# HKUST-Aerial-Robotics/Omni-swarm

Measured on NVIDIA H100. Metric: keyframes/sec (SuperPoint+NetVLAD+match), higher is better.
Workload: dtype f32

## Files before the change

omni-swarm_b200/csrc/conv_umma.cu:

```cuda
#include <cuda.h>
#include <cuda_fp16.h>
#include <cmath>
#include "common.cuh"
#include "kernels.cuh"
#include "conv_umma.cuh"
#include "umma_ptx.cuh"

namespace osb {

constexpr int UM_TH = 8, UM_TW = 16;
constexpr int UM_KC = 64;
constexpr int UM_ROW = UM_TW * 128;

constexpr int UM_A_SLOT = (UM_TH + 2) * UM_ROW;
constexpr int UM_A_SLOTS = 2;
constexpr int UM_CONSUMERS = 256;
constexpr int UM_THREADS = UM_CONSUMERS + 128;
constexpr int UM_PRODUCER_REGS = 40, UM_CONSUMER_REGS = 232;
static_assert(128 * UM_PRODUCER_REGS + UM_CONSUMERS * UM_CONSUMER_REGS <= 65536, "register file");
template <int N, bool FP16 = false>
struct UmmaCfg {
  static constexpr int PLANES = FP16 ? 1 : 2;
  static constexpr int A_SLOTS = FP16 ? 4 : UM_A_SLOTS;
  static constexpr int A_RING = A_SLOTS * PLANES * UM_A_SLOT;
  static constexpr int B_BYTES = N * 128;
  static constexpr int B_SLOT = PLANES * B_BYTES;
  static constexpr int B_SLOTS = FP16 ? ((N <= 64) ? 12 : (N <= 80) ? 10 : 8) : ((N <= 64) ? 6 : (N <= 80) ? 5 : 4);
  static constexpr int SMEM_BYTES = A_RING + B_SLOTS * B_SLOT + 1024  + 256 ;
  static_assert(SMEM_BYTES <= 227 * 1024, "shared-memory plan exceeds the 227 KB of an H100 block");
  static_assert(2 * (A_SLOTS + B_SLOTS) * 8 <= 256, "barriers exceed their 256 bytes");
};
template <bool FP16 = false>
struct R64Cfg {
  static constexpr int PLANES = FP16 ? 1 : 2;
  static constexpr int A_SLOTS = FP16 ? 6 : UM_A_SLOTS;
  static constexpr int A_RING = A_SLOTS * PLANES * UM_A_SLOT;
  static constexpr int W_PLANE = 64 * 128;
  static constexpr int W_SLOT = PLANES * W_PLANE;
  static constexpr int SMEM_BYTES = A_RING + 9 * W_SLOT + 1024  + 256 ;
  static_assert(SMEM_BYTES <= 227 * 1024, "shared-memory plan exceeds the 227 KB of an H100 block");
  static_assert((3 * A_SLOTS + 9) * 8 <= 256, "barriers exceed their 256 bytes");
};

struct UmmaArgs {
  const float* bias;
  __half* out_hi;
  __half* out_lo;
  float* out_f32;
  int H, W, B;
  int ks;
  int cin_slabs;
  int out_c;
  int out_cstride;
  float inv_scale;
  float out_scale;
  int relu;
  int n_off;
  int pool;
  int n_split;
  int epi;
};

__device__ __forceinline__ void quad_transpose(uint32_t (&v)[4], int t4) {
  uint32_t o[4];
#pragma unroll
  for (int k = 0; k < 4; ++k) o[k] = (k == t4) ? v[k] : 0u;
#pragma unroll
  for (int r = 1; r < 4; ++r) {
    const int send = (t4 - r) & 3, from = (t4 + r) & 3;
    uint32_t s = v[0];
#pragma unroll
    for (int k = 1; k < 4; ++k) s = (send == k) ? v[k] : s;
    const uint32_t got = __shfl_sync(0xffffffffu, s, (threadIdx.x & 28) | from);
#pragma unroll
    for (int k = 0; k < 4; ++k) o[k] = (from == k) ? got : o[k];
  }
#pragma unroll
  for (int k = 0; k < 4; ++k) v[k] = o[k];
}

template <int N, bool SPLIT, bool FP16 = false>
__global__ void __launch_bounds__(UM_THREADS, 1)
conv_umma_kernel(const __grid_constant__ CUtensorMap tm_a_hi, const __grid_constant__ CUtensorMap tm_a_lo,
                 const __grid_constant__ CUtensorMap tm_w_hi, const __grid_constant__ CUtensorMap tm_w_lo, UmmaArgs P) {
  using Cfg = UmmaCfg<N, FP16>;
  constexpr int AS = Cfg::A_SLOTS, BS = Cfg::B_SLOTS, A_STRIDE = Cfg::PLANES * UM_A_SLOT;
  extern __shared__ uint8_t smem_raw[];
  const uint32_t smem_base = (smem_u32(smem_raw) + 1023u) & ~1023u;
  const uint32_t b_base = smem_base + Cfg::A_RING;
  const uint32_t bar_base = b_base + BS * Cfg::B_SLOT;
  auto a_full = [&](int s) { return bar_base + 8u * s; };
  auto a_empty = [&](int s) { return bar_base + 8u * (AS + s); };
  auto b_full = [&](int s) { return bar_base + 8u * (2 * AS + s); };
  auto b_empty = [&](int s) { return bar_base + 8u * (2 * AS + BS + s); };

  const int lane = threadIdx.x & 31;
  const int tiles_x = (P.W + UM_TW - 1) / UM_TW, tiles_y = (P.H + UM_TH - 1) / UM_TH;
  const int n_tiles = P.B * tiles_x * tiles_y;
  const int n_split = SPLIT ? P.n_split : 1;
  const int n_items = n_tiles * n_split;
  const int halo = P.ks / 2;
  const uint32_t a_box_bytes = (uint32_t)(UM_TH + 2 * halo) * UM_ROW;

  if (threadIdx.x == 0) {
    for (int s = 0; s < AS; ++s) { mbar_init(a_full(s), 1); mbar_init(a_empty(s), 2); }
    for (int s = 0; s < BS; ++s) { mbar_init(b_full(s), 1); mbar_init(b_empty(s), 2); }
    asm volatile("fence.mbarrier_init.release.cluster;" ::: "memory");
  }
  __syncthreads();
  asm volatile("griddepcontrol.launch_dependents;" ::: "memory");

  if (threadIdx.x >= UM_CONSUMERS) {
    const int pt = threadIdx.x - UM_CONSUMERS;
    setmaxnreg_dec<UM_PRODUCER_REGS>();
    asm volatile("griddepcontrol.wait;" ::: "memory");
    if (pt < 32 && elect_one()) {
      int as = 0; uint32_t aph = 0;
      int bs = 0; uint32_t bph = 0;
      for (int item = blockIdx.x; item < n_items; item += gridDim.x) {
        const int tile = SPLIT ? item / n_split : item, n_off = SPLIT ? P.n_off + (item % n_split) * N : P.n_off;
        const int tx = tile % tiles_x, ty = (tile / tiles_x) % tiles_y, b = tile / (tiles_x * tiles_y);
        const int x0 = tx * UM_TW, y0 = ty * UM_TH;
        for (int kx = 0; kx < P.ks; ++kx) {
          for (int cs = 0; cs < P.cin_slabs; ++cs) {
            mbar_wait(a_empty(as), aph ^ 1);
            const uint32_t sa = smem_base + as * A_STRIDE;
            mbar_expect_tx(a_full(as), Cfg::PLANES * a_box_bytes);
            tma_load_4d(sa, &tm_a_hi, a_full(as), cs * UM_KC, x0 + kx - halo, y0 - halo, b);
            if constexpr (!FP16) tma_load_4d(sa + UM_A_SLOT, &tm_a_lo, a_full(as), cs * UM_KC, x0 + kx - halo, y0 - halo, b);
            if (++as == AS) { as = 0; aph ^= 1; }
            for (int ky = 0; ky < P.ks; ++ky) {
              mbar_wait(b_empty(bs), bph ^ 1);
              const uint32_t sb = b_base + bs * Cfg::B_SLOT;
              mbar_expect_tx(b_full(bs), Cfg::B_SLOT);
              tma_load_3d(sb, &tm_w_hi, b_full(bs), cs * UM_KC, n_off, ky * P.ks + kx);
              if constexpr (!FP16) tma_load_3d(sb + Cfg::B_BYTES, &tm_w_lo, b_full(bs), cs * UM_KC, n_off, ky * P.ks + kx);
              if (++bs == BS) { bs = 0; bph ^= 1; }
            }
          }
        }
      }
    }
  } else {
    setmaxnreg_inc<UM_CONSUMER_REGS>();
    const int cw = threadIdx.x >> 7;
    const int wq = (threadIdx.x >> 5) & 3;
    const int col = lane >> 2, t4 = lane & 3;
    const bool signaller = (threadIdx.x & 127) == 0;
    int as = 0; uint32_t aph = 0;
    int bs = 0; uint32_t bph = 0;
    auto release = [&](int a_slot, int b_slot) {
      if (!signaller) return;
      if (a_slot >= 0) mbar_arrive(a_empty(a_slot));
      if (b_slot >= 0) mbar_arrive(b_empty(b_slot));
    };
    for (int item = blockIdx.x; item < n_items; item += gridDim.x) {
      const int tile = SPLIT ? item / n_split : item, n_off = SPLIT ? P.n_off + (item % n_split) * N : P.n_off;
      float acc[N / 2], cross[FP16 ? 1 : N / 2];
#pragma unroll
      for (int i = 0; i < N / 2; ++i) { acc[i] = 0.f; if constexpr (!FP16) cross[i] = 0.f; }
      uint32_t scale_d = 0;
      int pend_a = -1, pend_b = -1;
      for (int kx = 0; kx < P.ks; ++kx) {
        for (int cs = 0; cs < P.cin_slabs; ++cs) {
          mbar_wait(a_full(as), aph);
          const uint32_t sa = smem_base + as * A_STRIDE + cw * 1024;
          for (int ky = 0; ky < P.ks; ++ky) {
            mbar_wait(b_full(bs), bph);
            const uint32_t sb = b_base + bs * Cfg::B_SLOT;
            const int b_slot = bs;
            if (++bs == BS) { bs = 0; bph ^= 1; }
            const uint64_t a_hi = wgmma_desc_sw128(sa + ky * UM_ROW, UM_ROW);
            const uint64_t a_lo = wgmma_desc_sw128(sa + UM_A_SLOT + ky * UM_ROW, UM_ROW);
            const uint64_t b_hi = wgmma_desc_sw128(sb, 1024), b_lo = wgmma_desc_sw128(sb + Cfg::B_BYTES, 1024);
#pragma unroll
            for (int i = 0; i < N / 2; ++i) { fence_operand(acc[i]); if constexpr (!FP16) fence_operand(cross[i]); }
            wgmma_fence();
#pragma unroll
            for (int k = 0; k < UM_KC / 16; ++k) {
              const uint64_t adv = (uint64_t)(k * 32 >> 4);
// ... 126 lines not shown
          float f[4];
#pragma unroll
          for (int i = 0; i < 4; ++i) {
            float a = value(4 * j + i, c + (i & 1));
            if (P.relu) a = fmaxf(a, 0.f);
            if (P.relu == 2) a = fminf(a, 6.f);
            f[i] = a;
          }
          if (P.pool) {
            float m0 = fmaxf(f[0], f[2]), m1 = fmaxf(f[1], f[3]);
            m0 = fmaxf(m0, __shfl_xor_sync(0xffffffffu, m0, 4));
            m1 = fmaxf(m1, __shfl_xor_sync(0xffffffffu, m1, 4));
            if (pool_writer) store(ppix, c, m0, m1);
          } else {
            if (in0) store(pix0, c, f[0], f[1]);
            if (in1) store(pix1, c, f[2], f[3]);
          }
        }
      }
    }
  }
}

template <bool FP16 = false>
__global__ void __launch_bounds__(UM_THREADS, 1)
conv_res64_kernel(const __grid_constant__ CUtensorMap tm_a_hi, const __grid_constant__ CUtensorMap tm_a_lo,
                  const __grid_constant__ CUtensorMap tm_w_hi, const __grid_constant__ CUtensorMap tm_w_lo, UmmaArgs P) {
  using Cfg = R64Cfg<FP16>;
  constexpr int AS = Cfg::A_SLOTS, A_STRIDE = Cfg::PLANES * UM_A_SLOT;
  constexpr int R64_W_PLANE = Cfg::W_PLANE, R64_W_SLOT = Cfg::W_SLOT;
  extern __shared__ uint8_t smem_raw[];
  const uint32_t smem_base = (smem_u32(smem_raw) + 1023u) & ~1023u;
  const uint32_t w_base = smem_base + Cfg::A_RING;
  const uint32_t bar_base = w_base + 9 * R64_W_SLOT;
  auto a_full = [&](int g, int s) { return bar_base + 8u * (g * AS + s); };
  auto a_empty = [&](int s) { return bar_base + 8u * (2 * AS + s); };
  auto w_full = [&](int t) { return bar_base + 8u * (3 * AS + t); };

  const int lane = threadIdx.x & 31;
  const int tiles_x = (P.W + UM_TW - 1) / UM_TW, tiles_y = (P.H + UM_TH - 1) / UM_TH;
  const int n_tiles = P.B * tiles_x * tiles_y;

  if (threadIdx.x == 0) {
    for (int s = 0; s < AS; ++s) { mbar_init(a_full(0, s), 1); mbar_init(a_full(1, s), 1); mbar_init(a_empty(s), 1); }
    for (int t = 0; t < 9; ++t) mbar_init(w_full(t), 1);
    asm volatile("fence.mbarrier_init.release.cluster;" ::: "memory");
// ... 60 lines not shown
#pragma unroll
          for (int k = 0; k < UM_KC / 16; ++k) {
            const uint64_t adv = (uint64_t)(k * 32 >> 4);
            Wgmma<128>::mma(acc, w_hi + adv, x_hi + adv, scale_d);
            if constexpr (!FP16) {
              Wgmma<128>::mma(cross, w_lo + adv, x_hi + adv, scale_d);
              Wgmma<128>::mma(cross, w_hi + adv, x_lo + adv, 1u);
            }
            scale_d = 1;
          }
          wgmma_commit();
#pragma unroll
          for (int k = 0; k < 64; ++k) { fence_operand(acc[k]); if constexpr (!FP16) fence_operand(cross[k]); }
          wgmma_wait<1>();
          if (signaller && pend >= 0) mbar_arrive(a_empty(pend));
          pend = (ky == 2) ? as : -1;
        }
      }
      wgmma_wait<0>();
      if (signaller) mbar_arrive(a_empty(pend));
#pragma unroll
      for (int k = 0; k < 64; ++k) { fence_operand(acc[k]); if constexpr (!FP16) fence_operand(cross[k]); }

      const int tx = tile % tiles_x, ty = (tile / tiles_x) % tiles_y, b = tile / (tiles_x * tiles_y);
      const int x0 = tx * UM_TW, y0 = ty * UM_TH;
      auto value = [&](int k, int h) {
        float a;
        if constexpr (FP16) a = fmaf(acc[k], P.inv_scale, bias[h]);
        else a = fmaf(acc[k] + cross[k], P.inv_scale, bias[h]);
        if (P.relu) a = fmaxf(a, 0.f);
        if (P.relu == 2) a = fminf(a, 6.f);
        return a;
      };
      auto split_t = [&](float v0, float v1, uint32_t& th, uint32_t& tl) {
        const float s0 = v0 * P.out_scale, s1 = v1 * P.out_scale;
        const __half2 hp = __floats2half2_rn(s0, s1);
        if constexpr (FP16) {
          th = movmatrix_trans(*reinterpret_cast<const uint32_t*>(&hp));
        } else {
          const float2 hf = __half22float2(hp);
          const __half2 lp = __floats2half2_rn(s0 - hf.x, s1 - hf.y);
          th = movmatrix_trans(*reinterpret_cast<const uint32_t*>(&hp));
          tl = movmatrix_trans(*reinterpret_cast<const uint32_t*>(&lp));
        }
      };
#pragma unroll
      for (int h = 0; h < 2; ++h) {
        const int cb = 16 * w + 8 * h;
        if (cb >= P.out_c) continue;
        const int c_own = P.n_off + cb + r, c_st = P.n_off + cb + 2 * t4;
        if (P.pool) {
          const int Hp = P.H >> 1, Wp = P.W >> 1;
#pragma unroll
          for (int py = 0; py < UM_TH / 2; ++py) {
            float m[2];
#pragma unroll
            for (int k = 0; k < 2; ++k) {
              const int j = 4 * py + k;
              m[k] = fmaxf(fmaxf(value(4 * j + 2 * h, h), value(4 * (j + 2) + 2 * h, h)),
                           fmaxf(value(4 * j + 2 * h + 1, h), value(4 * (j + 2) + 2 * h + 1, h)));
            }
            const int gpy = ty * (UM_TH / 2) + py;
            if (P.out_f32) {
#pragma unroll
              for (int k = 0; k < 2; ++k) {
                const int gpx = tx * (UM_TW / 2) + 4 * k + t4;
                if (gpy < Hp && gpx < Wp)
                  P.out_f32[(((size_t)b * Hp + gpy) * Wp + gpx) * P.out_cstride + c_own] = m[k];
              }
            } else {
              uint32_t th, tl;
              split_t(m[0], m[1], th, tl);
              const int gpx = tx * (UM_TW / 2) + 4 * (r & 1) + (r >> 1);
              if (gpy < Hp && gpx < Wp) {
                const size_t o = (((size_t)b * Hp + gpy) * Wp + gpx) * P.out_cstride + c_st;
                *reinterpret_cast<uint32_t*>(P.out_hi + o) = th;
                if constexpr (!FP16) *reinterpret_cast<uint32_t*>(P.out_lo + o) = tl;
              }
            }
          }
        } else {
#pragma unroll
          for (int j = 0; j < 16; ++j) {
            const int gy = y0 + (j >> 1), xb = x0 + 8 * (j & 1);
            const float v0 = value(4 * j + 2 * h, h), v1 = value(4 * j + 2 * h + 1, h);
            if (P.out_f32) {
              const int gx = xb + 2 * t4;
              const size_t o = (((size_t)b * P.H + gy) * P.W + gx) * P.out_cstride + c_own;
              if (gy < P.H && gx < P.W) P.out_f32[o] = v0;
              if (gy < P.H && gx + 1 < P.W) P.out_f32[o + P.out_cstride] = v1;
            } else {
              uint32_t th, tl;
              split_t(v0, v1, th, tl);
              const int gx = xb + r;
              if (gy < P.H && gx < P.W) {
                const size_t o = (((size_t)b * P.H + gy) * P.W + gx) * P.out_cstride + c_st;
                *reinterpret_cast<uint32_t*>(P.out_hi + o) = th;
                if constexpr (!FP16) *reinterpret_cast<uint32_t*>(P.out_lo + o) = tl;
              }
            }
          }
        }
      }
    }
  }
}

template <bool FP16>
__device__ __forceinline__ void split_store8(__half* hi, __half* lo, const float* f, float scale) {
  uint32_t h[4], l[4];
#pragma unroll
  for (int i = 0; i < 4; ++i) {
    const float s0 = f[2 * i] * scale, s1 = f[2 * i + 1] * scale;
    const __half h0 = __float2half_rn(s0), h1 = __float2half_rn(s1);
    h[i] = (uint32_t)__half_as_ushort(h0) | ((uint32_t)__half_as_ushort(h1) << 16);
    if constexpr (!FP16) {
      const __half l0 = __float2half_rn(s0 - __half2float(h0)), l1 = __float2half_rn(s1 - __half2float(h1));
      l[i] = (uint32_t)__half_as_ushort(l0) | ((uint32_t)__half_as_ushort(l1) << 16);
    }
  }
  *reinterpret_cast<uint4*>(hi) = make_uint4(h[0], h[1], h[2], h[3]);
  if constexpr (!FP16) *reinterpret_cast<uint4*>(lo) = make_uint4(l[0], l[1], l[2], l[3]);
}

constexpr int CF_TW = 32, CF_TH = 8;
template <bool FP16 = false>
// ... 110 lines not shown
    bp[o] = bias[o];
    for (int c = 0; c < cin; ++c)
      for (int t = 0; t < L->taps; ++t) {
        const float s = w_oihw[((size_t)o * cin + c) * L->taps + t] * w_scale;
        const __half h = __float2half_rn(s);
        if (!std::isfinite(__half2float(h))) {
          char buf[192];
          snprintf(buf, sizeof(buf), "weight %g (output %d, input %d, tap %d) is outside the split-fp16 range: "
                   "|w| * %g must be below 65520", (double)w_oihw[((size_t)o * cin + c) * L->taps + t], o, c, t,
                   (double)w_scale);
          set_error("umma_layer_upload", buf);
          return OSB_ERR_INVALID;
        }
        const size_t idx = ((size_t)t * L->n_pad + o) * cin + c;
        hi[idx] = h;
        lo[idx] = __float2half_rn(s - __half2float(h));
      }
  }
  OSB_TRY(res.upload(&L->w_hi, hi.data(), n));
  OSB_TRY(res.upload(&L->w_lo, lo.data(), n));
  OSB_TRY(res.upload(&L->bias, bp.data(), L->n_pad));
  const uint64_t dims[3] = {(uint64_t)cin, (uint64_t)L->n_pad, (uint64_t)L->taps};
  const uint64_t strides[2] = {(uint64_t)cin * 2, (uint64_t)cin * L->n_pad * 2};
  const uint32_t box[3] = {UM_KC, (uint32_t)std::min(L->n_pad, 256), 1};
  OSB_TRY(umma_make_tmap(&L->tm_hi, L->w_hi, 3, dims, strides, box));
  OSB_TRY(umma_make_tmap(&L->tm_lo, L->w_lo, 3, dims, strides, box));
  if (L->n_pad >= 256) {
    const uint32_t box128[3] = {UM_KC, 128, 1};
    OSB_TRY(umma_make_tmap(&L->tm_hi128, L->w_hi, 3, dims, strides, box128));
    OSB_TRY(umma_make_tmap(&L->tm_lo128, L->w_lo, 3, dims, strides, box128));
  }
  return OSB_OK;
}

osb_status umma_act_maps(CUtensorMap* hi, CUtensorMap* lo, __half* p_hi, __half* p_lo, int B, int H, int W, int C,
                         int ks) {
  const uint64_t dims[4] = {(uint64_t)C, (uint64_t)W, (uint64_t)H, (uint64_t)B};
  const uint64_t strides[3] = {(uint64_t)C * 2, (uint64_t)W * C * 2, (uint64_t)H * W * C * 2};
  const uint32_t box[4] = {UM_KC, UM_TW, (uint32_t)(UM_TH + 2 * (ks / 2)), 1};
  osb_status s;
  if ((s = umma_make_tmap(hi, p_hi, 4, dims, strides, box)) != OSB_OK) return s;
  return umma_make_tmap(lo, p_lo, 4, dims, strides, box);
}

static const bool g_conv_pdl = [] { const char* e = getenv("OSB_CONV_PDL"); return e && atoi(e) != 0; }();

template <auto kernel>
static osb_status launch_persistent(int smem_bytes, const CUtensorMap& a_hi, const CUtensorMap& a_lo,
                                    const CUtensorMap& w_hi, const CUtensorMap& w_lo, const UmmaArgs& P, cudaStream_t st,
                                    int max_ctas) {
  OSB_SMEM_OPT_IN(kernel, smem_bytes);
  const int tiles = P.B * cdiv(P.W, UM_TW) * cdiv(P.H, UM_TH) * P.n_split;
  const int grid = std::min(tiles, persistent_ctas(max_ctas));
  cudaLaunchConfig_t cfg = {};
  cudaLaunchAttribute attr[1];
  cfg.gridDim = dim3(grid); cfg.blockDim = dim3(UM_THREADS); cfg.dynamicSmemBytes = smem_bytes; cfg.stream = st;
  attr[0].id = cudaLaunchAttributeProgrammaticStreamSerialization;
  attr[0].val.programmaticStreamSerializationAllowed = g_conv_pdl ? 1 : 0;
  cfg.attrs = attr; cfg.numAttrs = 1;
  OSB_CUDA(cudaLaunchKernelEx(&cfg, kernel, a_hi, a_lo, w_hi, w_lo, P));
  g_launches.fetch_add(1, std::memory_order_relaxed);
  return OSB_OK;
}

template <int N, bool SPLIT = false, bool FP16 = false>
static osb_status launch_umma(const CUtensorMap& a_hi, const CUtensorMap& a_lo, const UmmaLayer& L, const UmmaArgs& P,
                              cudaStream_t st, int max_ctas, bool box128 = false) {
  return launch_persistent<conv_umma_kernel<N, SPLIT, FP16>>(UmmaCfg<N, FP16>::SMEM_BYTES, a_hi, a_lo,
                           box128 ? L.tm_hi128 : L.tm_hi, box128 ? L.tm_lo128 : L.tm_lo, P, st, max_ctas);
}

static bool precision_fp16(int precision) { return precision == OSB_PRECISION_FP16; }

static UmmaArgs umma_args(const UmmaLayer& L, int B, int H, int W, float act_scale) {
  UmmaArgs P = {};
  P.bias = L.bias; P.H = H; P.W = W; P.B = B; P.ks = L.ks; P.cin_slabs = L.cin / UM_KC;
  P.inv_scale = 1.0f / (act_scale * L.w_scale); P.n_split = 1;
  return P;
}

template <bool FP16>
static osb_status umma_conv_launch(const UmmaLayer& L, const CUtensorMap& a_hi, const CUtensorMap& a_lo, UmmaArgs& P,
                                   cudaStream_t st, int max_ctas) {
  switch (L.n_pad) {
    case 64:
      if (L.ks == 3 && L.cin == UM_KC)
        return launch_persistent<conv_res64_kernel<FP16>>(R64Cfg<FP16>::SMEM_BYTES, a_hi, a_lo, L.tm_hi, L.tm_lo, P, st,
                                                          max_ctas);
      return launch_umma<64, false, FP16>(a_hi, a_lo, L, P, st, max_ctas);
    case 80: return launch_umma<80, false, FP16>(a_hi, a_lo, L, P, st, max_ctas);
    case 128: return launch_umma<128, false, FP16>(a_hi, a_lo, L, P, st, max_ctas);
    case 256:
    case 512:
      P.n_split = L.n_pad / 128;
      return launch_umma<128, true, FP16>(a_hi, a_lo, L, P, st, max_ctas, true);
  }
  set_error("umma_conv_forward", "unsupported N");
  return OSB_ERR_INVALID;
}

osb_status umma_conv_forward(const UmmaLayer& L, const CUtensorMap& a_hi, const CUtensorMap& a_lo, int B, int H, int W,
                             float act_scale, __half* out_hi, __half* out_lo, float* out_f32, int out_c, int out_cstride,
                             float out_scale, int relu, int pool, cudaStream_t st, int max_ctas, int precision) {
  OSB_REQUIRE(!pool || (H % 2 == 0 && W % 2 == 0), "fused max-pool needs even H and W");
  OSB_REQUIRE(out_c % 16 == 0 && out_c <= L.n_pad && out_cstride % 8 == 0, "tensor-core conv: bad output channel layout");
  UmmaArgs P = umma_args(L, B, H, W, act_scale);
  P.out_hi = out_hi; P.out_lo = out_lo; P.out_f32 = out_f32; P.out_c = out_c; P.out_cstride = out_cstride;
  P.out_scale = out_scale; P.relu = relu; P.pool = pool;
  return precision_fp16(precision) ? umma_conv_launch<true>(L, a_hi, a_lo, P, st, max_ctas)
                                   : umma_conv_launch<false>(L, a_hi, a_lo, P, st, max_ctas);
}

osb_status umma_conv_softmax_forward(const UmmaLayer& L, const CUtensorMap& a_hi, const CUtensorMap& a_lo, int B, int H, int W,
                                     float act_scale, float* semi, cudaStream_t st, int max_ctas, int precision) {
  OSB_REQUIRE(L.n_pad == 80 && L.cout == 65 && L.ks == 1, "fused detector head expects the 65-logit 1x1 layer");
  UmmaArgs P = umma_args(L, B, H, W, act_scale);
  P.out_f32 = semi; P.out_c = 80; P.out_cstride = 80; P.out_scale = 1.f; P.epi = 1;
  return precision_fp16(precision) ? launch_umma<80, false, true>(a_hi, a_lo, L, P, st, max_ctas)
                                   : launch_umma<80>(a_hi, a_lo, L, P, st, max_ctas);
}

template <bool FP16 = false>
__global__ void dwconv3x3_split_kernel(const float* __restrict__ w, const float* __restrict__ bias,
                                       const float* __restrict__ x, __half* __restrict__ out_hi,
                                       __half* __restrict__ out_lo, int H, int W, int Ho, int Wo, int C, int stride,
                                       float out_scale, int64_t total) {
  const int64_t i = (int64_t)blockIdx.x * blockDim.x + threadIdx.x;
  if (i >= total) return;
  const int C8 = C >> 3;
  const int c = (int)(i % C8) * 8;
  int64_t p = i / C8;
  const int ox = (int)(p % Wo); p /= Wo;
  const int oy = (int)(p % Ho);
  const int b = (int)(p / Ho);
  float a[8];
#pragma unroll
  for (int j = 0; j < 8; ++j) a[j] = 0.f;
#pragma unroll
  for (int ky = 0; ky < 3; ++ky)
#pragma unroll
    for (int kx = 0; kx < 3; ++kx) {
// ... 230 lines not shown
```

omni-swarm_b200/csrc/conv_umma.cuh:

```cuda
#pragma once
#include <cuda.h>
#include <cuda_fp16.h>
#include "common.cuh"

namespace osb {

struct UmmaLayer {
  int cin = 0, cout = 0, n_pad = 0, ks = 1, taps = 1;
  float w_scale = 1.f;
  __half *w_hi = nullptr, *w_lo = nullptr;
  float* bias = nullptr;
  CUtensorMap tm_hi, tm_lo;
  CUtensorMap tm_hi128, tm_lo128;
};

osb_status umma_layer_upload(Resources& res, UmmaLayer* L, const float* w_oihw, const float* bias, int cin, int cout,
                             int ks, float w_scale);
osb_status umma_act_maps(CUtensorMap* hi, CUtensorMap* lo, __half* p_hi, __half* p_lo, int B, int H, int W, int C,
                         int ks);
osb_status umma_conv_forward(const UmmaLayer& L, const CUtensorMap& a_hi, const CUtensorMap& a_lo, int B, int H, int W,
                             float act_scale, __half* out_hi, __half* out_lo, float* out_f32, int out_c, int out_cstride,
                             float out_scale, int relu, int pool, cudaStream_t st, int max_ctas = 0,
                             int precision = OSB_PRECISION_SPLIT_FP16);
osb_status umma_conv_softmax_forward(const UmmaLayer& L, const CUtensorMap& a_hi, const CUtensorMap& a_lo, int B, int H, int W,
                                     float act_scale, float* semi, cudaStream_t st, int max_ctas = 0,
                                     int precision = OSB_PRECISION_SPLIT_FP16);
osb_status umma_first_forward(const float* w_tap_cout, const float* bias, const float* lut, const uint8_t* img,
                              __half* out_hi, __half* out_lo, int B, int H, int W, float out_scale, cudaStream_t st,
                              int precision = OSB_PRECISION_SPLIT_FP16);
osb_status umma_make_tmap(CUtensorMap* tm, void* base, int rank, const uint64_t* dims, const uint64_t* strides_bytes,
                          const uint32_t* box);
osb_status umma_dwconv_forward(const float* w_tap_c, const float* bias, const float* x, __half* out_hi, __half* out_lo,
                               int B, int H, int W, int C, int stride, float out_scale, cudaStream_t st, bool s1x4 = true,
                               int precision = OSB_PRECISION_SPLIT_FP16);
}
```

omni-swarm_b200/csrc/umma_ptx.cuh:

```cuda
#pragma once
#include <cuda.h>
#include <cuda_fp16.h>
#include <stdint.h>

namespace osb {

__device__ __forceinline__ uint32_t smem_u32(const void* p) { return (uint32_t)__cvta_generic_to_shared(p); }
__device__ __forceinline__ void mbar_init(uint32_t bar, uint32_t count) {
  asm volatile("mbarrier.init.shared::cta.b64 [%0], %1;" ::"r"(bar), "r"(count) : "memory");
}
__device__ __forceinline__ void mbar_expect_tx(uint32_t bar, uint32_t bytes) {
  asm volatile("mbarrier.arrive.expect_tx.shared::cta.b64 _, [%0], %1;" ::"r"(bar), "r"(bytes) : "memory");
}
__device__ __forceinline__ void mbar_arrive(uint32_t bar) {
  asm volatile("mbarrier.arrive.shared::cta.b64 _, [%0];" ::"r"(bar) : "memory");
}
__device__ __forceinline__ void mbar_wait(uint32_t bar, uint32_t parity) {
  uint32_t done;
  uint32_t spins = 0;
  do {
    asm volatile("{\n\t.reg .pred p;\n\tmbarrier.try_wait.parity.shared::cta.b64 p, [%1], %2;\n\tselp.u32 %0, 1, 0, p;\n\t}"
                 : "=r"(done) : "r"(bar), "r"(parity) : "memory");
#ifdef OSB_MBAR_DEBUG
    if (!done && ++spins > (1u << 22)) {
      if (blockIdx.x == 0 && (threadIdx.x & 31) == 0)
        printf("mbar_wait stalled: block %d thread %d barrier +%u parity %u\n", blockIdx.x, threadIdx.x, bar & 0xFFFFu, parity);
      return;
    }
#else
    if (!done && ++spins > (1u << 24)) __trap();
#endif
  } while (!done);
}
__device__ __forceinline__ void tma_load_4d(uint32_t dst, const CUtensorMap* tm, uint32_t bar, int c0, int c1, int c2, int c3) {
  asm volatile("cp.async.bulk.tensor.4d.shared::cluster.global.tile.mbarrier::complete_tx::bytes [%0], [%1, {%3, %4, %5, %6}], [%2];"
               ::"r"(dst), "l"(tm), "r"(bar), "r"(c0), "r"(c1), "r"(c2), "r"(c3) : "memory");
}
__device__ __forceinline__ void tma_load_3d(uint32_t dst, const CUtensorMap* tm, uint32_t bar, int c0, int c1, int c2) {
  asm volatile("cp.async.bulk.tensor.3d.shared::cluster.global.tile.mbarrier::complete_tx::bytes [%0], [%1, {%3, %4, %5}], [%2];"
               ::"r"(dst), "l"(tm), "r"(bar), "r"(c0), "r"(c1), "r"(c2) : "memory");
}
__device__ __forceinline__ bool elect_one() {
  uint32_t pred = 0;
  asm volatile("{\n\t.reg .pred p;\n\telect.sync _|p, 0xffffffff;\n\tselp.u32 %0, 1, 0, p;\n\t}" : "=r"(pred));
  return pred != 0;
}

__device__ __forceinline__ uint64_t wgmma_desc_sw128(uint32_t saddr, uint32_t sbo_bytes) {
  return (uint64_t)((saddr >> 4) & 0x3FFF) | (1ull << 16) | ((uint64_t)((sbo_bytes >> 4) & 0x3FFF) << 32) | (1ull << 62);
}
template <int R> __device__ __forceinline__ void setmaxnreg_dec() { asm volatile("setmaxnreg.dec.sync.aligned.u32 %0;" ::"n"(R)); }
template <int R> __device__ __forceinline__ void setmaxnreg_inc() { asm volatile("setmaxnreg.inc.sync.aligned.u32 %0;" ::"n"(R)); }
__device__ __forceinline__ void wgmma_fence() { asm volatile("wgmma.fence.sync.aligned;" ::: "memory"); }
__device__ __forceinline__ void wgmma_commit() { asm volatile("wgmma.commit_group.sync.aligned;" ::: "memory"); }
template <int N> __device__ __forceinline__ void wgmma_wait() { asm volatile("wgmma.wait_group.sync.aligned %0;" ::"n"(N) : "memory"); }
__device__ __forceinline__ void fence_operand(float& r) { asm volatile("" : "+f"(r)::"memory"); }
__device__ __forceinline__ uint32_t movmatrix_trans(uint32_t a) {
  uint32_t d;
  asm volatile("movmatrix.sync.aligned.m8n8.trans.b16 %0, %1;" : "=r"(d) : "r"(a));
  return d;
}

template <int W> struct Wgmma;
template <> struct Wgmma<64> {
  static __device__ __forceinline__ void mma(float* d, uint64_t a, uint64_t b, uint32_t scale_d) {
    asm volatile("{\n\t.reg .pred p;\n\tsetp.ne.b32 p, %34, 0;\n\t"
                 "wgmma.mma_async.sync.aligned.m64n64k16.f32.f16.f16 {%0, %1, %2, %3, %4, %5, %6, %7, %8, %9, %10, %11, %12, %13, %14, %15, %16, %17, %18, %19, %20, %21, %22, %23, %24, %25, %26, %27, %28, %29, %30, %31}, %32, %33, p, 1, 1, 0, 0;\n\t}"
                 : "+f"(d[0]), "+f"(d[1]), "+f"(d[2]), "+f"(d[3]), "+f"(d[4]), "+f"(d[5]), "+f"(d[6]), "+f"(d[7]), "+f"(d[8]), "+f"(d[9]), "+f"(d[10]), "+f"(d[11]), "+f"(d[12]), "+f"(d[13]), "+f"(d[14]), "+f"(d[15]), "+f"(d[16]), "+f"(d[17]), "+f"(d[18]), "+f"(d[19]), "+f"(d[20]), "+f"(d[21]), "+f"(d[22]), "+f"(d[23]), "+f"(d[24]), "+f"(d[25]), "+f"(d[26]), "+f"(d[27]), "+f"(d[28]), "+f"(d[29]), "+f"(d[30]), "+f"(d[31])
                 : "l"(a), "l"(b), "r"(scale_d));
  }
// ... 21 lines not shown
```

Baseline: 363.6.

## Add transposed-stream conv kernel for 128+ channel layers with per-warpgroup weight rings

After: 385.1, median of 6. +5.9%, better.

```diff
diff --git a/omni-swarm_b200/csrc/conv_umma.cu b/omni-swarm_b200/csrc/conv_umma.cu
--- a/omni-swarm_b200/csrc/conv_umma.cu
+++ b/omni-swarm_b200/csrc/conv_umma.cu
@@ -20,12 +20,13 @@
 static_assert(128 * UM_PRODUCER_REGS + UM_CONSUMERS * UM_CONSUMER_REGS <= 65536, "register file");
 template <int N, bool FP16 = false>
 struct UmmaCfg {
+  static_assert(N == 64 || N == 80, "128-channel layers run in conv_stream_t_kernel");
   static constexpr int PLANES = FP16 ? 1 : 2;
   static constexpr int A_SLOTS = FP16 ? 4 : UM_A_SLOTS;
   static constexpr int A_RING = A_SLOTS * PLANES * UM_A_SLOT;
   static constexpr int B_BYTES = N * 128;
   static constexpr int B_SLOT = PLANES * B_BYTES;
-  static constexpr int B_SLOTS = FP16 ? ((N <= 64) ? 12 : (N <= 80) ? 10 : 8) : ((N <= 64) ? 6 : (N <= 80) ? 5 : 4);
+  static constexpr int B_SLOTS = FP16 ? ((N <= 64) ? 12 : 10) : ((N <= 64) ? 6 : 5);
   static constexpr int SMEM_BYTES = A_RING + B_SLOTS * B_SLOT + 1024  + 256 ;
   static_assert(SMEM_BYTES <= 227 * 1024, "shared-memory plan exceeds the 227 KB of an H100 block");
   static_assert(2 * (A_SLOTS + B_SLOTS) * 8 <= 256, "barriers exceed their 256 bytes");
@@ -40,6 +41,19 @@
   static constexpr int SMEM_BYTES = A_RING + 9 * W_SLOT + 1024  + 256 ;
   static_assert(SMEM_BYTES <= 227 * 1024, "shared-memory plan exceeds the 227 KB of an H100 block");
   static_assert((3 * A_SLOTS + 9) * 8 <= 256, "barriers exceed their 256 bytes");
+};
+template <bool FP16 = false>
+struct StreamTCfg {
+  static constexpr int PLANES = FP16 ? 1 : 2;
+  static constexpr int A_SLOTS = FP16 ? 6 : 3;
+  static constexpr int A_RING = A_SLOTS * PLANES * UM_A_SLOT;
+  static constexpr int W_PLANE = 64 * 128;
+  static constexpr int W_SLOT = PLANES * W_PLANE;
+  static constexpr int W_SLOTS = FP16 ? 6 : 3;
+  static constexpr int SMEM_BYTES = A_RING + 2 * W_SLOTS * W_SLOT + 1024  + 512 ;
+  static_assert(A_SLOTS >= 3 && W_SLOTS >= 3, "the rings need three slots each for the two warpgroups to run apart");
+  static_assert(SMEM_BYTES <= 227 * 1024, "shared-memory plan exceeds the 227 KB of an H100 block");
+  static_assert(2 * (A_SLOTS + 2 * W_SLOTS) * 8 <= 512, "barriers exceed their 512 bytes");
 };
 
 struct UmmaArgs {
@@ -79,7 +93,7 @@
   for (int k = 0; k < 4; ++k) v[k] = o[k];
 }
 
-template <int N, bool SPLIT, bool FP16 = false>
+template <int N, bool FP16 = false>
 __global__ void __launch_bounds__(UM_THREADS, 1)
 conv_umma_kernel(const __grid_constant__ CUtensorMap tm_a_hi, const __grid_constant__ CUtensorMap tm_a_lo,
                  const __grid_constant__ CUtensorMap tm_w_hi, const __grid_constant__ CUtensorMap tm_w_lo, UmmaArgs P) {
@@ -97,8 +111,6 @@
   const int lane = threadIdx.x & 31;
   const int tiles_x = (P.W + UM_TW - 1) / UM_TW, tiles_y = (P.H + UM_TH - 1) / UM_TH;
   const int n_tiles = P.B * tiles_x * tiles_y;
-  const int n_split = SPLIT ? P.n_split : 1;
-  const int n_items = n_tiles * n_split;
   const int halo = P.ks / 2;
   const uint32_t a_box_bytes = (uint32_t)(UM_TH + 2 * halo) * UM_ROW;
 
@@ -117,8 +129,7 @@
     if (pt < 32 && elect_one()) {
       int as = 0; uint32_t aph = 0;
       int bs = 0; uint32_t bph = 0;
-      for (int item = blockIdx.x; item < n_items; item += gridDim.x) {
-        const int tile = SPLIT ? item / n_split : item, n_off = SPLIT ? P.n_off + (item % n_split) * N : P.n_off;
+      for (int tile = blockIdx.x; tile < n_tiles; tile += gridDim.x) {
         const int tx = tile % tiles_x, ty = (tile / tiles_x) % tiles_y, b = tile / (tiles_x * tiles_y);
         const int x0 = tx * UM_TW, y0 = ty * UM_TH;
         for (int kx = 0; kx < P.ks; ++kx) {
@@ -133,8 +144,8 @@
               mbar_wait(b_empty(bs), bph ^ 1);
               const uint32_t sb = b_base + bs * Cfg::B_SLOT;
               mbar_expect_tx(b_full(bs), Cfg::B_SLOT);
-              tma_load_3d(sb, &tm_w_hi, b_full(bs), cs * UM_KC, n_off, ky * P.ks + kx);
-              if constexpr (!FP16) tma_load_3d(sb + Cfg::B_BYTES, &tm_w_lo, b_full(bs), cs * UM_KC, n_off, ky * P.ks + kx);
+              tma_load_3d(sb, &tm_w_hi, b_full(bs), cs * UM_KC, P.n_off, ky * P.ks + kx);
+              if constexpr (!FP16) tma_load_3d(sb + Cfg::B_BYTES, &tm_w_lo, b_full(bs), cs * UM_KC, P.n_off, ky * P.ks + kx);
               if (++bs == BS) { bs = 0; bph ^= 1; }
             }
           }
@@ -154,8 +165,8 @@
       if (a_slot >= 0) mbar_arrive(a_empty(a_slot));
       if (b_slot >= 0) mbar_arrive(b_empty(b_slot));
     };
-    for (int item = blockIdx.x; item < n_items; item += gridDim.x) {
-      const int tile = SPLIT ? item / n_split : item, n_off = SPLIT ? P.n_off + (item % n_split) * N : P.n_off;
+    const int n_off = P.n_off;
+    for (int tile = blockIdx.x; tile < n_tiles; tile += gridDim.x) {
       float acc[N / 2], cross[FP16 ? 1 : N / 2];
 #pragma unroll
       for (int i = 0; i < N / 2; ++i) { acc[i] = 0.f; if constexpr (!FP16) cross[i] = 0.f; }
@@ -328,6 +339,100 @@
   }
 }
 
+template <bool FP16>
+__device__ __forceinline__ void tr_epilogue(const float (&acc)[64], const float (&cross)[FP16 ? 1 : 64],
+                                            const float (&bias)[2], int c_abs, int c_rel, int tile, int tiles_x,
+                                            int tiles_y, const UmmaArgs& P, int w, int r, int t4) {
+  if (c_rel + 16 * w >= P.out_c) return;
+  const int tx = tile % tiles_x, ty = (tile / tiles_x) % tiles_y, b = tile / (tiles_x * tiles_y);
+  const int x0 = tx * UM_TW, y0 = ty * UM_TH;
+  auto value = [&](int k, int h) {
+    float a;
+    if constexpr (FP16) a = fmaf(acc[k], P.inv_scale, bias[h]);
+    else a = fmaf(acc[k] + cross[k], P.inv_scale, bias[h]);
+    if (P.relu) a = fmaxf(a, 0.f);
+    if (P.relu == 2) a = fminf(a, 6.f);
+    return a;
+  };
+  auto split_t = [&](float v0, float v1, uint32_t& th, uint32_t& tl) {
+    const float s0 = v0 * P.out_scale, s1 = v1 * P.out_scale;
+    const __half2 hp = __floats2half2_rn(s0, s1);
+    if constexpr (FP16) {
+      th = movmatrix_trans(*reinterpret_cast<const uint32_t*>(&hp));
+    } else {
+      const float2 hf = __half22float2(hp);
+      const __half2 lp = __floats2half2_rn(s0 - hf.x, s1 - hf.y);
+      th = movmatrix_trans(*reinterpret_cast<const uint32_t*>(&hp));
+      tl = movmatrix_trans(*reinterpret_cast<const uint32_t*>(&lp));
+    }
+  };
+  if (!P.pool && !P.out_f32) {
+#pragma unroll
+    for (int y = 0; y < UM_TH; ++y) {
+      uint32_t th[4], tl[4];
+#pragma unroll
+      for (int k = 0; k < 4; ++k) {
+        const int j = 2 * y + (k >> 1), h = k & 1;
+        split_t(value(4 * j + 2 * h, h), value(4 * j + 2 * h + 1, h), th[k], tl[k]);
+      }
+      quad_transpose(th, t4);
+      if constexpr (!FP16) quad_transpose(tl, t4);
+      const int gy = y0 + y, gx = x0 + 8 * (t4 >> 1) + r;
+      if (gy < P.H && gx < P.W) {
+        const size_t o = (((size_t)b * P.H + gy) * P.W + gx) * P.out_cstride + c_abs + 16 * w + 8 * (t4 & 1);
+        *reinterpret_cast<uint4*>(P.out_hi + o) = make_uint4(th[0], th[1], th[2], th[3]);
+        if constexpr (!FP16) *reinterpret_cast<uint4*>(P.out_lo + o) = make_uint4(tl[0], tl[1], tl[2], tl[3]);
+      }
+    }
+    return;
+  }
+#pragma unroll
+  for (int h = 0; h < 2; ++h) {
+    const int cb = 16 * w + 8 * h;
+    const int c_own = c_abs + cb + r, c_st = c_abs + cb + 2 * t4;
+    if (P.pool) {
+      const int Hp = P.H >> 1, Wp = P.W >> 1;
+#pragma unroll
+      for (int py = 0; py < UM_TH / 2; ++py) {
+        float m[2];
+#pragma unroll
+        for (int k = 0; k < 2; ++k) {
+          const int j = 4 * py + k;
+          m[k] = fmaxf(fmaxf(value(4 * j + 2 * h, h), value(4 * (j + 2) + 2 * h, h)),
+                       fmaxf(value(4 * j + 2 * h + 1, h), value(4 * (j + 2) + 2 * h + 1, h)));
+        }
+        const int gpy = ty * (UM_TH / 2) + py;
+        if (P.out_f32) {
+#pragma unroll
+          for (int k = 0; k < 2; ++k) {
+            const int gpx = tx * (UM_TW / 2) + 4 * k + t4;
+            if (gpy < Hp && gpx < Wp) P.out_f32[(((size_t)b * Hp + gpy) * Wp + gpx) * P.out_cstride + c_own] = m[k];
+          }
+        } else {
+          uint32_t th, tl;
+          split_t(m[0], m[1], th, tl);
+          const int gpx = tx * (UM_TW / 2) + 4 * (r & 1) + (r >> 1);
+          if (gpy < Hp && gpx < Wp) {
+            const size_t o = (((size_t)b * Hp + gpy) * Wp + gpx) * P.out_cstride + c_st;
+            *reinterpret_cast<uint32_t*>(P.out_hi + o) = th;
+            if constexpr (!FP16) *reinterpret_cast<uint32_t*>(P.out_lo + o) = tl;
+          }
+        }
+      }
+    } else {
+#pragma unroll
+      for (int j = 0; j < 16; ++j) {
+        const uint32_t u0 = __float_as_uint(value(4 * j + 2 * h, h)), u1 = __float_as_uint(value(4 * j + 2 * h + 1, h));
+        const uint32_t tlo = movmatrix_trans(__byte_perm(u0, u1, 0x5410)), thi = movmatrix_trans(__byte_perm(u0, u1, 0x7632));
+        const int gy = y0 + (j >> 1), gx = x0 + 8 * (j & 1) + r;
+        if (gy < P.H && gx < P.W)
+          *reinterpret_cast<float2*>(P.out_f32 + (((size_t)b * P.H + gy) * P.W + gx) * P.out_cstride + c_st) =
+              make_float2(__uint_as_float(__byte_perm(tlo, thi, 0x5410)), __uint_as_float(__byte_perm(tlo, thi, 0x7632)));
+      }
+    }
+  }
+}
+
 template <bool FP16 = false>
 __global__ void __launch_bounds__(UM_THREADS, 1)
 conv_res64_kernel(const __grid_constant__ CUtensorMap tm_a_hi, const __grid_constant__ CUtensorMap tm_a_lo,
@@ -434,86 +539,143 @@
 #pragma unroll
       for (int k = 0; k < 64; ++k) { fence_operand(acc[k]); if constexpr (!FP16) fence_operand(cross[k]); }
 
-      const int tx = tile % tiles_x, ty = (tile / tiles_x) % tiles_y, b = tile / (tiles_x * tiles_y);
-      const int x0 = tx * UM_TW, y0 = ty * UM_TH;
-      auto value = [&](int k, int h) {
-        float a;
-        if constexpr (FP16) a = fmaf(acc[k], P.inv_scale, bias[h]);
-        else a = fmaf(acc[k] + cross[k], P.inv_scale, bias[h]);
-        if (P.relu) a = fmaxf(a, 0.f);
-        if (P.relu == 2) a = fminf(a, 6.f);
-        return a;
-      };
-      auto split_t = [&](float v0, float v1, uint32_t& th, uint32_t& tl) {
-        const float s0 = v0 * P.out_scale, s1 = v1 * P.out_scale;
-        const __half2 hp = __floats2half2_rn(s0, s1);
-        if constexpr (FP16) {
-          th = movmatrix_trans(*reinterpret_cast<const uint32_t*>(&hp));
-        } else {
-          const float2 hf = __half22float2(hp);
-          const __half2 lp = __floats2half2_rn(s0 - hf.x, s1 - hf.y);
-          th = movmatrix_trans(*reinterpret_cast<const uint32_t*>(&hp));
-          tl = movmatrix_trans(*reinterpret_cast<const uint32_t*>(&lp));
-        }
-      };
-#pragma unroll
-      for (int h = 0; h < 2; ++h) {
-        const int cb = 16 * w + 8 * h;
-        if (cb >= P.out_c) continue;
-        const int c_own = P.n_off + cb + r, c_st = P.n_off + cb + 2 * t4;
-        if (P.pool) {
-          const int Hp = P.H >> 1, Wp = P.W >> 1;
-#pragma unroll
-          for (int py = 0; py < UM_TH / 2; ++py) {
-            float m[2];
-#pragma unroll
-            for (int k = 0; k < 2; ++k) {
-              const int j = 4 * py + k;
-              m[k] = fmaxf(fmaxf(value(4 * j + 2 * h, h), value(4 * (j + 2) + 2 * h, h)),
-                           fmaxf(value(4 * j + 2 * h + 1, h), value(4 * (j + 2) + 2 * h + 1, h)));
+      tr_epilogue<FP16>(acc, cross, bias, P.n_off, 0, tile, tiles_x, tiles_y, P, w, r, t4);
+    }
+  }
+}
+
+template <bool SPLIT, bool FP16 = false>
+__global__ void __launch_bounds__(UM_THREADS, 1)
+conv_stream_t_kernel(const __grid_constant__ CUtensorMap tm_a_hi, const __grid_constant__ CUtensorMap tm_a_lo,
+                     const __grid_constant__ CUtensorMap tm_w_hi, const __grid_constant__ CUtensorMap tm_w_lo, UmmaArgs P) {
+  using Cfg = StreamTCfg<FP16>;
+  constexpr int AS = Cfg::A_SLOTS, WS = Cfg::W_SLOTS, A_STRIDE = Cfg::PLANES * UM_A_SLOT;
+  extern __shared__ uint8_t smem_raw[];
+  const uint32_t smem_base = (smem_u32(smem_raw) + 1023u) & ~1023u;
+  const uint32_t w_base = smem_base + Cfg::A_RING;
+  const uint32_t bar_base = w_base + 2 * WS * Cfg::W_SLOT;
+  auto a_full = [&](int s) { return bar_base + 8u * s; };
+  auto a_empty = [&](int s) { return bar_base + 8u * (AS + s); };
+  auto w_full = [&](int g, int s) { return bar_base + 8u * (2 * AS + g * WS + s); };
+  auto w_empty = [&](int g, int s) { return bar_base + 8u * (2 * AS + 2 * WS + g * WS + s); };
+
+  const int lane = threadIdx.x & 31;
+  const int tiles_x = (P.W + UM_TW - 1) / UM_TW, tiles_y = (P.H + UM_TH - 1) / UM_TH;
+  const int n_split = SPLIT ? P.n_split : 1;
+  const int n_items = P.B * tiles_x * tiles_y * n_split;
+  const int halo = P.ks / 2;
+  const uint32_t a_box_bytes = (uint32_t)(UM_TH + 2 * halo) * UM_ROW;
+
+  if (threadIdx.x == 0) {
+    for (int s = 0; s < AS; ++s) { mbar_init(a_full(s), 1); mbar_init(a_empty(s), 2); }
+    for (int s = 0; s < 2 * WS; ++s) { mbar_init(w_full(0, s), 1); mbar_init(w_empty(0, s), 1); }
+    asm volatile("fence.mbarrier_init.release.cluster;" ::: "memory");
+  }
+  __syncthreads();
+  asm volatile("griddepcontrol.launch_dependents;" ::: "memory");
+
+  if (threadIdx.x >= UM_CONSUMERS) {
+    const int pw = (threadIdx.x - UM_CONSUMERS) >> 5;
+    setmaxnreg_dec<UM_PRODUCER_REGS>();
+    asm volatile("griddepcontrol.wait;" ::: "memory");
+    if (pw < 3 && elect_one()) {
+      const int g = pw - 1;
+      int s = 0; uint32_t ph = 0;
+      for (int item = blockIdx.x; item < n_items; item += gridDim.x) {
+        const int tile = SPLIT ? item / n_split : item, n_off = SPLIT ? P.n_off + (item % n_split) * 128 : P.n_off;
+        const int tx = tile % tiles_x, ty = (tile / tiles_x) % tiles_y, b = tile / (tiles_x * tiles_y);
+        for (int kx = 0; kx < P.ks; ++kx) {
+          for (int cs = 0; cs < P.cin_slabs; ++cs) {
+            if (pw == 0) {
+              mbar_wait(a_empty(s), ph ^ 1);
+              const uint32_t sa = smem_base + s * A_STRIDE;
+              const int xa = tx * UM_TW + kx - halo, ya = ty * UM_TH - halo;
+              mbar_expect_tx(a_full(s), Cfg::PLANES * a_box_bytes);
+              tma_load_4d(sa, &tm_a_hi, a_full(s), cs * UM_KC, xa, ya, b);
+              if constexpr (!FP16) tma_load_4d(sa + UM_A_SLOT, &tm_a_lo, a_full(s), cs * UM_KC, xa, ya, b);
+              if (++s == AS) { s = 0; ph ^= 1; }
+              continue;
             }
-            const int gpy = ty * (UM_TH / 2) + py;
-            if (P.out_f32) {
-#pragma unroll
-              for (int k = 0; k < 2; ++k) {
-                const int gpx = tx * (UM_TW / 2) + 4 * k + t4;
-                if (gpy < Hp && gpx < Wp)
-                  P.out_f32[(((size_t)b * Hp + gpy) * Wp + gpx) * P.out_cstride + c_own] = m[k];
-              }
-            } else {
-              uint32_t th, tl;
-              split_t(m[0], m[1], th, tl);
-              const int gpx = tx * (UM_TW / 2) + 4 * (r & 1) + (r >> 1);
-              if (gpy < Hp && gpx < Wp) {
-                const size_t o = (((size_t)b * Hp + gpy) * Wp + gpx) * P.out_cstride + c_st;
-                *reinterpret_cast<uint32_t*>(P.out_hi + o) = th;
-                if constexpr (!FP16) *reinterpret_cast<uint32_t*>(P.out_lo + o) = tl;
-              }
+            for (int ky = 0; ky < P.ks; ++ky) {
+              mbar_wait(w_empty(g, s), ph ^ 1);
+              const uint32_t sw = w_base + (g * WS + s) * Cfg::W_SLOT;
+              mbar_expect_tx(w_full(g, s), Cfg::W_SLOT);
+              tma_load_3d(sw, &tm_w_hi, w_full(g, s), cs * UM_KC, n_off + 64 * g, ky * P.ks + kx);
+              if constexpr (!FP16)
+                tma_load_3d(sw + Cfg::W_PLANE, &tm_w_lo, w_full(g, s), cs * UM_KC, n_off + 64 * g, ky * P.ks + kx);
+              if (++s == WS) { s = 0; ph ^= 1; }
             }
           }
-        } else {
-#pragma unroll
-          for (int j = 0; j < 16; ++j) {
-            const int gy = y0 + (j >> 1), xb = x0 + 8 * (j & 1);
-            const float v0 = value(4 * j + 2 * h, h), v1 = value(4 * j + 2 * h + 1, h);
-            if (P.out_f32) {
-              const int gx = xb + 2 * t4;
-              const size_t o = (((size_t)b * P.H + gy) * P.W + gx) * P.out_cstride + c_own;
-              if (gy < P.H && gx < P.W) P.out_f32[o] = v0;
-              if (gy < P.H && gx + 1 < P.W) P.out_f32[o + P.out_cstride] = v1;
-            } else {
-              uint32_t th, tl;
-              split_t(v0, v1, th, tl);
-              const int gx = xb + r;
-              if (gy < P.H && gx < P.W) {
-                const size_t o = (((size_t)b * P.H + gy) * P.W + gx) * P.out_cstride + c_st;
-                *reinterpret_cast<uint32_t*>(P.out_hi + o) = th;
-                if constexpr (!FP16) *reinterpret_cast<uint32_t*>(P.out_lo + o) = tl;
+        }
+      }
+    }
+  } else {
+    setmaxnreg_inc<UM_CONSUMER_REGS>();
+    const int g = threadIdx.x >> 7;
+    const int w = (threadIdx.x >> 5) & 3;
+    const int r = lane >> 2, t4 = lane & 3;
+    const bool signaller = (threadIdx.x & 127) == 0;
+    const uint32_t w_ring = w_base + g * WS * Cfg::W_SLOT;
+    bool skew_set = g == 1;
+    if (g == 1) named_bar_sync(1, 256);
+    auto release = [&](int a_slot, int w_slot) {
+      if (!signaller) return;
+      if (a_slot >= 0) mbar_arrive(a_empty(a_slot));
+      if (w_slot >= 0) mbar_arrive(w_empty(g, w_slot));
+    };
+    int as = 0; uint32_t aph = 0;
+    int ws = 0; uint32_t wph = 0;
+    for (int item = blockIdx.x; item < n_items; item += gridDim.x) {
+      const int tile = SPLIT ? item / n_split : item, n_off = SPLIT ? P.n_off + (item % n_split) * 128 : P.n_off;
+      const int c_abs = n_off + 64 * g;
+      const float bias[2] = {__ldg(P.bias + c_abs + 16 * w + r), __ldg(P.bias + c_abs + 16 * w + 8 + r)};
+      float acc[64], cross[FP16 ? 1 : 64];
+#pragma unroll
+      for (int k = 0; k < 64; ++k) { acc[k] = 0.f; if constexpr (!FP16) cross[k] = 0.f; }
+      uint32_t scale_d = 0;
+      int pend_a = -1, pend_w = -1;
+      for (int kx = 0; kx < P.ks; ++kx) {
+        for (int cs = 0; cs < P.cin_slabs; ++cs) {
+          mbar_wait(a_full(as), aph);
+          const uint32_t sa = smem_base + as * A_STRIDE;
+          for (int ky = 0; ky < P.ks; ++ky) {
+            mbar_wait(w_full(g, ws), wph);
+            const uint32_t sw = w_ring + ws * Cfg::W_SLOT;
+            const int w_slot = ws;
+            if (++ws == WS) { ws = 0; wph ^= 1; }
+            const uint64_t w_hi = wgmma_desc_sw128(sw, 1024), w_lo = wgmma_desc_sw128(sw + Cfg::W_PLANE, 1024);
+            const uint64_t x_hi = wgmma_desc_sw128(sa + ky * UM_ROW, 1024);
+            const uint64_t x_lo = wgmma_desc_sw128(sa + UM_A_SLOT + ky * UM_ROW, 1024);
+#pragma unroll
+            for (int k = 0; k < 64; ++k) { fence_operand(acc[k]); if constexpr (!FP16) fence_operand(cross[k]); }
+            wgmma_fence();
+#pragma unroll
+            for (int k = 0; k < UM_KC / 16; ++k) {
+              const uint64_t adv = (uint64_t)(k * 32 >> 4);
+              Wgmma<128>::mma(acc, w_hi + adv, x_hi + adv, scale_d);
+              if constexpr (!FP16) {
+                Wgmma<128>::mma(cross, w_lo + adv, x_hi + adv, scale_d);
+                Wgmma<128>::mma(cross, w_hi + adv, x_lo + adv, 1u);
               }
+              scale_d = 1;
             }
+            wgmma_commit();
+#pragma unroll
+            for (int k = 0; k < 64; ++k) { fence_operand(acc[k]); if constexpr (!FP16) fence_operand(cross[k]); }
+            wgmma_wait<1>();
+            release(pend_a, pend_w);
+            pend_a = (ky == P.ks - 1) ? as : -1;
+            pend_w = w_slot;
           }
-        }
-      }
+          if (++as == AS) { as = 0; aph ^= 1; }
+          if (!skew_set) { named_bar_arrive(1, 256); skew_set = true; }
+        }
+      }
+      wgmma_wait<0>();
+      release(pend_a, pend_w);
+#pragma unroll
+      for (int k = 0; k < 64; ++k) { fence_operand(acc[k]); if constexpr (!FP16) fence_operand(cross[k]); }
+      tr_epilogue<FP16>(acc, cross, bias, c_abs, c_abs - P.n_off, tile, tiles_x, tiles_y, P, w, r, t4);
     }
   }
 }
@@ -670,14 +832,9 @@
   OSB_TRY(res.upload(&L->bias, bp.data(), L->n_pad));
   const uint64_t dims[3] = {(uint64_t)cin, (uint64_t)L->n_pad, (uint64_t)L->taps};
   const uint64_t strides[2] = {(uint64_t)cin * 2, (uint64_t)cin * L->n_pad * 2};
-  const uint32_t box[3] = {UM_KC, (uint32_t)std::min(L->n_pad, 256), 1};
+  const uint32_t box[3] = {UM_KC, (uint32_t)(L->n_pad == 80 ? 80 : 64), 1};
   OSB_TRY(umma_make_tmap(&L->tm_hi, L->w_hi, 3, dims, strides, box));
   OSB_TRY(umma_make_tmap(&L->tm_lo, L->w_lo, 3, dims, strides, box));
-  if (L->n_pad >= 256) {
-    const uint32_t box128[3] = {UM_KC, 128, 1};
-    OSB_TRY(umma_make_tmap(&L->tm_hi128, L->w_hi, 3, dims, strides, box128));
-    OSB_TRY(umma_make_tmap(&L->tm_lo128, L->w_lo, 3, dims, strides, box128));
-  }
   return OSB_OK;
 }
 
@@ -711,11 +868,18 @@
   return OSB_OK;
 }
 
-template <int N, bool SPLIT = false, bool FP16 = false>
+template <int N, bool FP16 = false>
 static osb_status launch_umma(const CUtensorMap& a_hi, const CUtensorMap& a_lo, const UmmaLayer& L, const UmmaArgs& P,
-                              cudaStream_t st, int max_ctas, bool box128 = false) {
-  return launch_persistent<conv_umma_kernel<N, SPLIT, FP16>>(UmmaCfg<N, FP16>::SMEM_BYTES, a_hi, a_lo,
-                           box128 ? L.tm_hi128 : L.tm_hi, box128 ? L.tm_lo128 : L.tm_lo, P, st, max_ctas);
+                              cudaStream_t st, int max_ctas) {
+  return launch_persistent<conv_umma_kernel<N, FP16>>(UmmaCfg<N, FP16>::SMEM_BYTES, a_hi, a_lo, L.tm_hi, L.tm_lo, P, st,
+                                                      max_ctas);
+}
+
+template <bool SPLIT, bool FP16>
+static osb_status launch_stream_t(const CUtensorMap& a_hi, const CUtensorMap& a_lo, const UmmaLayer& L, const UmmaArgs& P,
+                                  cudaStream_t st, int max_ctas) {
+  return launch_persistent<conv_stream_t_kernel<SPLIT, FP16>>(StreamTCfg<FP16>::SMEM_BYTES, a_hi, a_lo, L.tm_hi, L.tm_lo,
+                                                              P, st, max_ctas);
 }
 
 static bool precision_fp16(int precision) { return precision == OSB_PRECISION_FP16; }
@@ -735,13 +899,13 @@
       if (L.ks == 3 && L.cin == UM_KC)
         return launch_persistent<conv_res64_kernel<FP16>>(R64Cfg<FP16>::SMEM_BYTES, a_hi, a_lo, L.tm_hi, L.tm_lo, P, st,
                                                           max_ctas);
-      return launch_umma<64, false, FP16>(a_hi, a_lo, L, P, st, max_ctas);
-    case 80: return launch_umma<80, false, FP16>(a_hi, a_lo, L, P, st, max_ctas);
-    case 128: return launch_umma<128, false, FP16>(a_hi, a_lo, L, P, st, max_ctas);
+      return launch_umma<64, FP16>(a_hi, a_lo, L, P, st, max_ctas);
+    case 80: return launch_umma<80, FP16>(a_hi, a_lo, L, P, st, max_ctas);
+    case 128: return launch_stream_t<false, FP16>(a_hi, a_lo, L, P, st, max_ctas);
     case 256:
     case 512:
       P.n_split = L.n_pad / 128;
-      return launch_umma<128, true, FP16>(a_hi, a_lo, L, P, st, max_ctas, true);
+      return launch_stream_t<true, FP16>(a_hi, a_lo, L, P, st, max_ctas);
   }
   set_error("umma_conv_forward", "unsupported N");
   return OSB_ERR_INVALID;
@@ -764,7 +928,7 @@
   OSB_REQUIRE(L.n_pad == 80 && L.cout == 65 && L.ks == 1, "fused detector head expects the 65-logit 1x1 layer");
   UmmaArgs P = umma_args(L, B, H, W, act_scale);
   P.out_f32 = semi; P.out_c = 80; P.out_cstride = 80; P.out_scale = 1.f; P.epi = 1;
-  return precision_fp16(precision) ? launch_umma<80, false, true>(a_hi, a_lo, L, P, st, max_ctas)
+  return precision_fp16(precision) ? launch_umma<80, true>(a_hi, a_lo, L, P, st, max_ctas)
                                    : launch_umma<80>(a_hi, a_lo, L, P, st, max_ctas);
 }
 
diff --git a/omni-swarm_b200/csrc/conv_umma.cuh b/omni-swarm_b200/csrc/conv_umma.cuh
--- a/omni-swarm_b200/csrc/conv_umma.cuh
+++ b/omni-swarm_b200/csrc/conv_umma.cuh
@@ -11,7 +11,6 @@
   __half *w_hi = nullptr, *w_lo = nullptr;
   float* bias = nullptr;
   CUtensorMap tm_hi, tm_lo;
-  CUtensorMap tm_hi128, tm_lo128;
 };
 
 osb_status umma_layer_upload(Resources& res, UmmaLayer* L, const float* w_oihw, const float* bias, int cin, int cout,
diff --git a/omni-swarm_b200/csrc/umma_ptx.cuh b/omni-swarm_b200/csrc/umma_ptx.cuh
--- a/omni-swarm_b200/csrc/umma_ptx.cuh
+++ b/omni-swarm_b200/csrc/umma_ptx.cuh
@@ -46,6 +46,13 @@
   return pred != 0;
 }
 
+__device__ __forceinline__ void named_bar_sync(uint32_t id, uint32_t count) {
+  asm volatile("bar.sync %0, %1;" ::"r"(id), "r"(count) : "memory");
+}
+__device__ __forceinline__ void named_bar_arrive(uint32_t id, uint32_t count) {
+  asm volatile("bar.arrive %0, %1;" ::"r"(id), "r"(count) : "memory");
+}
+
 __device__ __forceinline__ uint64_t wgmma_desc_sw128(uint32_t saddr, uint32_t sbo_bytes) {
   return (uint64_t)((saddr >> 4) & 0x3FFF) | (1ull << 16) | ((uint64_t)((sbo_bytes >> 4) & 0x3FFF) << 32) | (1ull << 62);
 }
```
